# hgyhungry/ge-spmm

Measured on AMD Instinct MI355X. Metric: SpMM GFLOP/s (= 2*nnz*N/t), CSR x dense fp32, N=128, higher is better.
Workload: dtype f32

## Files before the change

### gespmm_amd/csrc/plan.cpp

```cpp

#include <hip/hip_runtime.h>

#include <algorithm>
#include <atomic>
#include <chrono>
#include <cstdio>
#include <cstdlib>
#include <cstring>
#include <memory>
#include <new>
#include <vector>

#include "../../include/gespmm.h"
#include "auto_plan.h"
#include "plan.h"
#include "plan_device.h"
#include "plan_policy.h"
#include "reorder.h"
#include "sddmm_heads.h"
#include "select.h"
#include "spmm_device.h"
#include "spmm_heads.h"
#include "spmm_kernels.h"

// ... 141 lines not shown
void drop_plan_copy(gespmm_plan* p) {
    if (p->d_block) (void)hipFree(p->d_block);
    if (p->d_tasks) (void)hipFree(p->d_tasks);
    p->d_block = nullptr;
    p->d_perm = p->d_rowptr = p->d_colind = p->d_src_begin = p->d_tasks = p->d_gtasks = nullptr;
    p->d_val = nullptr;
    p->ntasks = p->ngtasks = 0;
}

hipError_t permute_values(const gespmm_plan* p, const float* val, hipStream_t st) {
    hipLaunchKernelGGL(permute_values_kernel, dim3((unsigned)((p->nnz + 255) / 256)), dim3(256), 0, st, p->d_rowptr, p->d_src_begin, val,
                       p->d_val, (int)p->M, (int)p->nnz);
    return hipGetLastError();
}

gespmm::ClusterOptions cluster_options_from_env() {
    gespmm::ClusterOptions o;
    if (const char* v = getenv("GESPMM_CLUSTER_LEVELS")) o.max_levels = atoi(v);
    if (const char* v = getenv("GESPMM_CLUSTER_SWEEPS")) o.sweeps = atoi(v);
    if (const char* v = getenv("GESPMM_CLUSTER_STOP")) o.stop_percent = atoi(v);
    if (const char* v = getenv("GESPMM_CLUSTER_CAP")) o.first_cap = atoi(v);
    return o;
}

gespmm::ClusterOptions cluster_options_for(const gespmm::PlanFacts& f, int threads) {
    gespmm::ClusterOptions o = cluster_options_from_env();
    if (o.max_levels <= 0) o.max_levels = gespmm::cluster_levels_for(f);
    if (o.sweeps <= 0) o.sweeps = gespmm::cluster_sweeps_for(f);
    o.threads = threads;
    return o;
}

void lap(hipStream_t st, const char* what) {
    static const bool timing = getenv("GESPMM_PLAN_TIMING") != nullptr;
    if (!timing) return;
    (void)hipStreamSynchronize(st);
    static thread_local std::chrono::steady_clock::time_point last;
    const auto now = std::chrono::steady_clock::now();
    if (what) fprintf(stderr, "[plan] %-22s %8.3f ms\n", what, std::chrono::duration<double>(now - last).count() * 1e3);
    last = now;
}

gespmm::RouteAnswer route_of(const gespmm_plan* p, int64_t N, int reduce, bool operands_aligned16) {
// ... 42 lines not shown
}

namespace gespmm {
bool plan_is_clustered(const gespmm_plan* p) { return p && p->reordered; }
static std::atomic<bool> g_analysis_warm{false};
bool analysis_is_warm() { return g_analysis_warm.load(std::memory_order_relaxed); }
void mark_analysis_warm() { g_analysis_warm.store(true, std::memory_order_relaxed); }
}

extern "C" {

int gespmm_cluster_rows(const int32_t* rowptr, const int32_t* colind, int64_t M, int64_t K, int32_t threads,
                        int32_t* perm_out, int32_t* levels_out, int32_t* clusters_out ) {
    if (M < 0 || K < 0 || (M > 0 && (!rowptr || !perm_out))) return GESPMM_EINVAL;
    gespmm::ClusterOptions opt;
    opt.threads = threads;
    gespmm::ClusterStats st;
    try {
        if (gespmm::cluster_rows(M, K, rowptr, colind, opt, perm_out, &st) != 0) return GESPMM_EINVAL;
    } catch (const std::bad_alloc&) {
        return GESPMM_ENOMEM;
    }
    if (levels_out) *levels_out = st.levels;
    if (clusters_out)
        for (int i = 0; i < 16; ++i) clusters_out[i] = st.clusters[i];
    return 0;
}

int gespmm_cluster_rows_study(const int32_t* rowptr, const int32_t* colind, int64_t M, int64_t K, int32_t max_levels, int32_t sweeps,
                              int32_t* perm_out, int32_t* top_label_out, int32_t* clusters_out ) {
// ... 19 lines not shown
}

int gespmm_device_cluster_rows(const int32_t* rowptr, const int32_t* colind, int64_t M, int64_t K, int64_t nnz,
                               int32_t* perm_out_host, int32_t* levels_out, int32_t* clusters_out , void* stream) {
    if (M < 0 || K < 0 || nnz < 0 || (M > 0 && (!rowptr || !perm_out_host)) || (nnz > 0 && !colind)) return GESPMM_EINVAL;
    if (M == 0) return 0;
    hipStream_t st = reinterpret_cast<hipStream_t>(stream);
    int32_t max_deg = 0, bad = 0;
    hipError_t e = gespmm::device_validate_csr(rowptr, colind, M, K, nnz, &max_deg, &bad, nullptr, st);
    if (e != hipSuccess) return (int)e;
    if (bad) return GESPMM_EINVAL;
    int32_t* d_perm = nullptr;
    e = hipMalloc(reinterpret_cast<void**>(&d_perm), (size_t)M * 4);
    if (e != hipSuccess) return (int)e;
    gespmm::ClusterOptions opt;
    gespmm::ClusterStats stats;
    e = gespmm::device_cluster_rows(M, K, nnz, rowptr, colind, opt, d_perm, &stats, st);
    if (e == hipSuccess) e = hipMemcpyAsync(perm_out_host, d_perm, (size_t)M * 4, hipMemcpyDeviceToHost, st);
    if (e == hipSuccess) e = hipStreamSynchronize(st);
    (void)hipFree(d_perm);
    if (e != hipSuccess) return (int)e;
    if (levels_out) *levels_out = stats.levels;
    if (clusters_out)
        for (int i = 0; i < 16; ++i) clusters_out[i] = stats.clusters[i];
    return 0;
}

double gespmm_device_l2_model(const int32_t* rowptr, const int32_t* colind, int64_t M, int64_t K, int64_t nnz,
                              const int32_t* perm_host, int32_t slices, int64_t window_rows, int64_t max_entries_per_slice,
                              int32_t samples_per_slice, void* stream) {
// ... 1001 lines not shown
    if (p->heads_last_route >= 0) {
        const size_t used = strlen(kern);
        char geo[64] = "";
        if (p->heads_last_route != 0)
            snprintf(geo, sizeof geo, " V=%d S=%d W=%d", p->heads_last_geo.vec, p->heads_last_geo.strips, p->heads_last_geo.group);
        snprintf(kern + used, sizeof kern - used, " | heads H=%lld F=%lld route=%d (%s%s)", (long long)p->heads_last_H, (long long)p->heads_last_F,
                 p->heads_last_route, p->heads_last_route == 1 ? (p->reordered ? "heads kernel, task table" : "heads kernel") : "per-head composition",
                 geo);
    }
    int n;
    if (p->reordered) {
        char lv[128] = "";
        int off = 0;
        for (int i = 0; i < p->stats.levels && i < 16 && off < 100; ++i)
            off += snprintf(lv + off, sizeof lv - (size_t)off, "%s%d", i ? ">" : "", p->stats.clusters[i]);
        char tuned[200] = "";
        if (p->tuned)
            snprintf(tuned, sizeof tuned, " tuned[us: batch-stream=%.1f segmented-stream=%.1f staged-rows=%.1f batch-stream-V4=%.1f padded-records=%.1f]",
                     p->tune_us[0], p->tune_us[1], p->tune_us[2], p->tune_us[3], p->tune_us[4]);
        n = snprintf(out, (size_t)capacity,
                     "order=%s levels=%d clusters=%s tasks=%d task_entries=%d group_tasks=%d max_degree=%d probe=%.3f l2_model=%.3f->%.3f "
                     "analysis=%.4fs on the %s (clustering %.4fs)%s | %s",
                     p->identity_order ? "storage(plan copy: as local as the clustering)" : "clustered", p->stats.levels, lv, p->ntasks, p->task_entries,
                     p->ngtasks, p->max_degree, p->facts.wedge_probe, p->hits_before,
                     p->hits_after, p->analysis_seconds, p->analysis == GESPMM_PLAN_ANALYSIS_HOST ? "host" : "device", p->cluster_seconds, tuned, kern);
    } else {
        char why[200] = "";
        if (p->cost_skipped)
            snprintf(why, sizeof why, " (analysis skipped: est. gain %.1f us x %d launches < est. cost %.0f us; wedge probe %.4f)", p->est_gain_us,
                     p->facts.expected_launches > 0 ? p->facts.expected_launches : gespmm::kDefaultExpectedLaunches, p->est_cost_us,
                     p->facts.wedge_probe);
        n = snprintf(out, (size_t)capacity, "order=storage max_degree=%d l2_model=%.3f->%.3f analysis=%.4fs%s | %s",
                     p->max_degree, p->hits_before, p->hits_after, p->analysis_seconds, why, kern);
    }
    return gespmm::describe_result(n, capacity);
}

void gespmm_release_cached_memory(void) { gespmm::release_cached_arena(); }
// ... 13 lines not shown
```

### gespmm_amd/csrc/plan_device.hip

```cpp

#include <hip/hip_runtime.h>
#include <stdint.h>

#include <algorithm>
#include <chrono>
#include <atomic>
#include <mutex>
#include <cstdio>
#include <cstdlib>
#include <vector>

#include <rocprim/device/device_radix_sort.hpp>
#include <rocprim/block/block_scan.hpp>
#include <rocprim/device/device_scan.hpp>
#include <rocprim/device/device_segmented_radix_sort.hpp>
#include <rocprim/functional.hpp>

#include "auto_plan.h"
#include "plan_device.h"
#include "spmm_device.h"
#include "spmm_kernels.h"
#include "workspace.h"

namespace gespmm {
// ... 347 lines not shown
    if (threadIdx.x < kBins) s_base[threadIdx.x] = s_cnt[threadIdx.x] > 0 ? atomicAdd(&counts[threadIdx.x], s_cnt[threadIdx.x]) : 0;
    __syncthreads();
    if (b >= 0) lists[(int64_t)b * n + s_base[b] + off] = i;
}

struct LpArgs {
    DAdj adj;
    const int32_t* nbr_label;
    const int32_t* cur;
    int32_t* next;
    const int32_t* size;
    const int32_t* rweight;
    long long cap;
    uint32_t seed;
    int skip_half;
    const int32_t* list;
    const int32_t* count;
    const int32_t* done;
};

__device__ inline bool sits_out(const LpArgs& a, int node) {
    return a.skip_half && (mix32((uint32_t)node * 0x85ebca6bu ^ a.seed) & 1u);
}

template <int G>
__device__ inline void best_of_group(long long& bt, uint32_t& bh, int& bL) {
#pragma unroll
    for (int o = G / 2; o > 0; o >>= 1) {
        const long long ot = __shfl_xor(bt, o, G);
        const uint32_t oh = (uint32_t)__shfl_xor((int)bh, o, G);
        const int oL = __shfl_xor(bL, o, G);
        if (ot > bt || (ot == bt && ot >= 0 && oh < bh)) {
            bt = ot;
            bh = oh;
// ... 15 lines not shown
        L = a.nbr_label[a.adj.idx[e]];
        wt = (L >= 0) ? (a.adj.w ? a.adj.w[e] : 1) : 0;
    }
    long long tot = 0;
#pragma unroll
    for (int j = 0; j < G; ++j) {
        const int Lj = __shfl(L, j, G);
        const int wj = __shfl(wt, j, G);
        tot += (Lj == L) ? wj : 0;
    }
    const int own = active ? a.cur[node] : -1;
    long long own_w = (L >= 0 && L == own) ? tot : 0;
#pragma unroll
    for (int o = G / 2; o > 0; o >>= 1) own_w = max(own_w, __shfl_xor(own_w, o, G));
    bool cand = L >= 0 && L != own && tot > own_w;
    if (ROWS && cand) cand = (long long)a.size[L] + a.rweight[node] <= a.cap;
    long long bt = cand ? tot : -1;
    uint32_t bh = mix32((uint32_t)L ^ a.seed);
    int bL = L;
    best_of_group<G>(bt, bh, bL);
    if (active && l == 0) a.next[node] = (ROWS && sits_out(a, node)) ? own : (bt >= 0 ? bL : own);
}

struct LpSmallClasses {
    const int32_t* lists;
    const int32_t* counts;
    int n_side;
    int blk_end[4];
};
template <bool ROWS>
// ... 48 lines not shown
        int slot = (int)(mix32((uint32_t)own) & (uint32_t)(T - 1));
        for (;;) {
            const int k = s_key[slot];
            if (k == own) {
                own_w = (long long)s_wt[slot];
                break;
            }
            if (k == -1) break;
            slot = (slot + 1) & (T - 1);
        }
    }
    long long bt = -1;
    uint32_t bh = 0;
    int bL = -1;
    const int rw = ROWS ? a.rweight[node] : 0;
    for (int s = lane; s < T; s += 64) {
        const int L = s_key[s];
        if (L < 0 || L == own) continue;
        const long long t = (long long)s_wt[s];
        if (t <= own_w) continue;
        if (ROWS && (long long)a.size[L] + rw > a.cap) continue;
        const uint32_t h = mix32((uint32_t)L ^ a.seed);
        if (t > bt || (t == bt && h < bh)) {
            bt = t;
            bh = h;
            bL = L;
        }
    }
    best_of_group<64>(bt, bh, bL);
    if (lane == 0) a.next[node] = bt >= 0 ? bL : own;
}

template <bool ROWS>
__global__ void __launch_bounds__(256) k_lp_dense(LpArgs a, unsigned long long* __restrict__ acc_all, int64_t nlabels) {
    __shared__ long long s_t[256];
// ... 11 lines not shown
            continue;
        }
        const int beg = a.adj.ptr[node], end = a.adj.ptr[node + 1];
        for (int e = beg + tid; e < end; e += 256) {
            const int L = a.nbr_label[a.adj.idx[e]];
            if (L >= 0) atomicAdd(&acc[L], (unsigned long long)(a.adj.w ? a.adj.w[e] : 1));
        }
        __threadfence();
        __syncthreads();
        const long long own_w =
            own >= 0 ? (long long)__hip_atomic_load(&acc[own], __ATOMIC_RELAXED, __HIP_MEMORY_SCOPE_AGENT) : 0;
        long long bt = -1;
        uint32_t bh = 0;
        int bL = -1;
        const int rw = ROWS ? a.rweight[node] : 0;
        for (int e = beg + tid; e < end; e += 256) {
            const int L = a.nbr_label[a.adj.idx[e]];
            if (L < 0 || L == own) continue;
            const long long t = (long long)__hip_atomic_load(&acc[L], __ATOMIC_RELAXED, __HIP_MEMORY_SCOPE_AGENT);
            if (t <= own_w) continue;
            if (ROWS && (long long)a.size[L] + rw > a.cap) continue;
            const uint32_t h = mix32((uint32_t)L ^ a.seed);
            if (t > bt || (t == bt && h < bh)) {
                bt = t;
                bh = h;
                bL = L;
            }
        }
        s_t[tid] = bt;
        s_h[tid] = bh;
        s_L[tid] = bL;
        __syncthreads();
        for (int o = 128; o > 0; o >>= 1) {
            if (tid < o) {
                const long long ot = s_t[tid + o];
// ... 12 lines not shown
            if (L >= 0) __hip_atomic_store(&acc[L], 0ull, __ATOMIC_RELAXED, __HIP_MEMORY_SCOPE_AGENT);
        }
        __threadfence();
        __syncthreads();
    }
}

__global__ void k_commit_cols(int32_t* __restrict__ cur, const int32_t* __restrict__ next, const int32_t* __restrict__ twin,
                              const int32_t* __restrict__ rlab, int n, const int32_t* __restrict__ done) {
    if (*done) return;
    const int i = blockIdx.x * blockDim.x + threadIdx.x;
    if (i < n) cur[i] = (twin && twin[i] >= 0) ? rlab[twin[i]] : next[i];
}

__global__ void k_commit_rows(int32_t* __restrict__ cur, const int32_t* __restrict__ next, const int32_t* __restrict__ rweight,
                              int32_t* __restrict__ size, int n, int32_t* __restrict__ changed, int32_t* __restrict__ ticket,
                              int32_t* __restrict__ done) {
    if (*done) return;
    const int i = blockIdx.x * blockDim.x + threadIdx.x;
    int ch = 0;
    if (i < n) {
        const int v = next[i], old = cur[i];
        if (v != old) {
            ch = 1;
            cur[i] = v;
            const int w = rweight[i];
            atomicAdd(&size[v], w);
            atomicSub(&size[old], w);
        }
    }
    __shared__ int s_changed;
    if (threadIdx.x == 0) s_changed = 0;
    __syncthreads();
    const unsigned long long m = __ballot(ch);
    if (m && lane_id() == (__ffsll((long long)m) - 1)) atomicAdd(&s_changed, __popcll(m));
    __syncthreads();
    if (threadIdx.x == 0) {
        if (s_changed) atomicAdd(changed, s_changed);
        __threadfence();
        if (atomicAdd(ticket, 1) == (int)gridDim.x - 1) {
            const int c = atomicAdd(changed, 0);
            if ((long long)c * 400 < n) atomicExch(done, 1);
            atomicExch(changed, 0);
            atomicExch(ticket, 0);
        }
    }
}


__global__ void k_mark_used(const int32_t* __restrict__ rlab, int R, const int32_t* __restrict__ clab, int C,
                            int32_t* __restrict__ used_r, int32_t* __restrict__ used_c) {
    const int i = blockIdx.x * blockDim.x + threadIdx.x;
    if (i < R) used_r[rlab[i]] = 1;
    if (i < C) {
        const int L = clab[i];
        if (L >= 0) used_c[L] = 1;
// ... 11 lines not shown

__global__ void k_level_init(int32_t* __restrict__ rlab, int32_t* __restrict__ rnext, int32_t* __restrict__ size,
                             const int32_t* __restrict__ rweight, int R, int32_t* __restrict__ clab,
                             int32_t* __restrict__ cnext, int C, int32_t* __restrict__ flags ) {
    const int i = blockIdx.x * blockDim.x + threadIdx.x;
    if (i < R) {
        rlab[i] = i;
        rnext[i] = i;
        size[i] = rweight[i];
    }
    if (i < C) {
        clab[i] = -1;
        cnext[i] = -1;
    }
    if (i < 16) flags[i] = 0;
}

__global__ void k_fill2(int32_t* __restrict__ a, int64_t na, int32_t va, int32_t* __restrict__ b, int64_t nb, int32_t vb) {
    const int64_t i = (int64_t)blockIdx.x * blockDim.x + threadIdx.x;
    if (i < na) a[i] = va;
    if (i < nb) b[i] = vb;
}

__global__ void k_parents(const int32_t* __restrict__ rlab, const int32_t* __restrict__ rid, int R,
                          int32_t* __restrict__ parent) {
    const int r = blockIdx.x * blockDim.x + threadIdx.x;
    if (r < R) parent[r] = rid[rlab[r]];
}

__global__ void k_new_weights(const int32_t* __restrict__ rlab, const int32_t* __restrict__ rid,
// ... 507 lines not shown
    lv.region = Scratch::kLevelA;
    GESPMM_TRY(build_cols(sc, lv, nullptr, st));
    {
        int32_t* rw = nullptr;
        sc.use(lv.region);
        GESPMM_TRY(sc.get(&rw, M));
        hipLaunchKernelGGL(k_fill, dim3(grid_for(M)), dim3(256), 0, st, rw, M, 1);
        lv.rweight = rw;
    }
    std::vector<int32_t*> parents;
    std::vector<int32_t> parent_count;
    std::vector<int32_t> cluster_count;

    int32_t* flags_dev = nullptr;
    static_assert(4 + 2 * kBins <= 16, "k_level_init zeroes 16 flags");
    sc.use(Scratch::kPersist);
    GESPMM_TRY(sc.get(&flags_dev, 16));

    long long cap = opt.first_cap > 0 ? opt.first_cap : 256;
    const int max_levels = opt.max_levels > 0 ? opt.max_levels : kDefaultClusterLevels;
    const int sweeps = opt.sweeps > 0 ? opt.sweeps : 5;
    const int stop_percent = opt.stop_percent > 0 ? opt.stop_percent : 97;

    static const bool timing = getenv("GESPMM_PLAN_TIMING") != nullptr;
    auto lap = [&](const char* what, int level) {
        if (!timing) return;
        (void)hipStreamSynchronize(st);
        static thread_local std::chrono::steady_clock::time_point last;
        const auto now = std::chrono::steady_clock::now();
        if (what) fprintf(stderr, "[plan]   L%d %-16s %8.3f ms\n", level, what, std::chrono::duration<double>(now - last).count() * 1e3);
        last = now;
    };
    lap(nullptr, 0);
    for (int level = 0; level < max_levels; ++level) {
        const int32_t R = lv.R, C = lv.C;
        if (R <= 1 || lv.E == 0) break;
        lap("(cols/setup)", level);
        sc.reset(Scratch::kTemp);
        sc.use(Scratch::kTemp);
        int32_t *rlab = nullptr, *clab = nullptr, *rnext = nullptr, *cnext = nullptr, *size = nullptr, *rlists = nullptr,
                *clists = nullptr;
        GESPMM_TRY(sc.get(&rlab, R));
        GESPMM_TRY(sc.get(&clab, C));
        const size_t after_labels = sc.mark();
        GESPMM_TRY(sc.get(&rnext, R));
        GESPMM_TRY(sc.get(&cnext, C));
        GESPMM_TRY(sc.get(&size, R));
        GESPMM_TRY(sc.get(&rlists, (int64_t)kBins * R));
        GESPMM_TRY(sc.get(&clists, (int64_t)kBins * C));
        hipLaunchKernelGGL(k_level_init, dim3(grid_for(std::max(R, C))), dim3(256), 0, st, rlab, rnext, size, lv.rweight, R, clab,
                           cnext, C, flags_dev);
        int32_t* done = flags_dev;
        int32_t* changed = flags_dev + 1;
        int32_t* ticket = flags_dev + 2;
        int32_t* rcounts = flags_dev + 4;
        int32_t* ccounts = flags_dev + 4 + kBins;
        hipLaunchKernelGGL(k_bin_nodes, dim3((unsigned)((R + kBinThreads - 1) / kBinThreads)), dim3(kBinThreads), 0, st, lv.rows.ptr,
                           (const int32_t*)nullptr, R, rlists, rcounts);
        hipLaunchKernelGGL(k_bin_nodes, dim3((unsigned)((C + kBinThreads - 1) / kBinThreads)), dim3(kBinThreads), 0, st, lv.cols.ptr,
                           lv.twin, C, clists, ccounts);
        GESPMM_TRY(hipGetLastError());
        int32_t h_counts[2 * kBins];
        GESPMM_TRY(fetch(h_counts, (const int32_t*)(flags_dev + 4), 2 * kBins, st));
        unsigned long long* acc = nullptr;
        int acc_wgs = 0;
        if (h_counts[kBins - 1] > 0 || h_counts[2 * kBins - 1] > 0) {
            const int want = std::max(h_counts[kBins - 1], h_counts[2 * kBins - 1]);
            int64_t wgs = std::min<int64_t>(want, 64);
            while (wgs > 1 && wgs * (int64_t)R * 8 > (1ll << 30)) wgs >>= 1;
            acc_wgs = (int)wgs;
            GESPMM_TRY(sc.get(&acc, (int64_t)acc_wgs * R));
            GESPMM_TRY(hipMemsetAsync(acc, 0, (size_t)acc_wgs * (size_t)R * 8, st));
        }
        const bool twins = lv.twin != nullptr;
        for (int sweep = 0; sweep < sweeps; ++sweep) {
            LpArgs a;
            a.seed = 0x9e3779b9u * (uint32_t)(level * 16 + sweep + 1);
            a.done = done;
            a.cap = cap;
            a.list = nullptr;
            a.count = nullptr;
            a.adj = lv.cols;
            a.nbr_label = rlab;
            a.cur = clab;
            a.next = cnext;
            a.size = nullptr;
            a.rweight = nullptr;
            a.skip_half = 0;
            GESPMM_TRY(launch_half_sweep<false>(a, clists, ccounts, h_counts + kBins, C, acc, acc_wgs, R, st));
            hipLaunchKernelGGL(k_commit_cols, dim3(grid_for(C)), dim3(256), 0, st, clab, (const int32_t*)cnext, lv.twin,
                               (const int32_t*)rlab, C, (const int32_t*)done);
            a.adj = lv.rows;
            a.nbr_label = clab;
            a.cur = rlab;
            a.next = rnext;
            a.size = size;
            a.rweight = lv.rweight;
            a.skip_half = (twins && sweep + 1 < sweeps) ? 1 : 0;
            GESPMM_TRY(launch_half_sweep<true>(a, rlists, rcounts, h_counts, R, acc, acc_wgs, R, st));
            hipLaunchKernelGGL(k_commit_rows, dim3((unsigned)((R + 1023) / 1024)), dim3(1024), 0, st, rlab, (const int32_t*)rnext,
                               lv.rweight, size, R, changed, ticket, done);
            GESPMM_TRY(hipGetLastError());
        }
        lap("sweeps", level);
        sc.rewind(Scratch::kTemp, after_labels);

        int32_t *used = nullptr, *pos = nullptr, *rid = nullptr, *cid = nullptr, *parent = nullptr;
        const int64_t R1 = (int64_t)R + 1;
        sc.use(Scratch::kPersist);
        GESPMM_TRY(sc.get(&parent, R));
        sc.use(Scratch::kTemp);
        GESPMM_TRY(sc.get(&rid, R));
        GESPMM_TRY(sc.get(&cid, R));
        const size_t after_ids = sc.mark();
        GESPMM_TRY(sc.get(&used, 2 * R1));
        GESPMM_TRY(sc.get(&pos, 2 * R1));
        GESPMM_TRY(hipMemsetAsync(used, 0, (size_t)(2 * R1) * 4, st));
        hipLaunchKernelGGL(k_mark_used, dim3(grid_for(std::max(R, C))), dim3(256), 0, st, (const int32_t*)rlab, R,
                           (const int32_t*)clab, C, used, used + R1);
        GESPMM_TRY(exclusive_scan<int32_t>(sc, used, pos, 2 * R1, st));
        hipLaunchKernelGGL(k_make_ids, dim3(grid_for(R)), dim3(256), 0, st, (const int32_t*)used, (const int32_t*)pos,
                           (const int32_t*)(pos + R), R, rid, cid);
        hipLaunchKernelGGL(k_parents, dim3(grid_for(R)), dim3(256), 0, st, (const int32_t*)rlab, (const int32_t*)rid, R, parent);
        GESPMM_TRY(hipGetLastError());
        int32_t tot[2] = {0, 0};
        GESPMM_TRY(hipMemcpyAsync(&tot[0], pos + R, 4, hipMemcpyDeviceToHost, st));
        GESPMM_TRY(hipMemcpyAsync(&tot[1], pos + 2 * R1 - 1, 4, hipMemcpyDeviceToHost, st));
        GESPMM_TRY(hipStreamSynchronize(st));
        const int32_t R2 = tot[0], C2 = tot[1] - tot[0];
        sc.rewind(Scratch::kTemp, after_ids);
        parents.push_back(parent);
        parent_count.push_back(R);
        cluster_count.push_back(R2);
        if (stats) {
            stats->levels = level + 1;
            if (level < 16) stats->clusters[level] = R2;
        }
        lap("relabel", level);
        const bool last = (R2 <= 8 || (int64_t)R2 * 100 > (int64_t)R * stop_percent || level + 1 >= max_levels);
        if (last) break;

        DLevel nx;
        nx.R = R2;
        nx.C = C2;
        nx.region = lv.region == Scratch::kLevelA ? Scratch::kLevelB : Scratch::kLevelA;
        sc.reset(nx.region);
        int32_t *rw2 = nullptr, *twin2 = nullptr;
        sc.use(nx.region);
        GESPMM_TRY(sc.get(&rw2, R2));
        GESPMM_TRY(sc.get(&twin2, C2));
        sc.use(Scratch::kTemp);
// ... 806 lines not shown
```

### gespmm_amd/csrc/plan_policy.cpp

```cpp

#include <cstdlib>
#include "plan_policy.h"

#include <cstddef>
#include <cstring>

#include "../../include/gespmm.h"
#include "select.h"
#include "spmm_kernels.h"

namespace gespmm {

int long_row_flags(int64_t M, int64_t nnz, int32_t max_degree, int user_flags) {
    const int64_t mean = M > 0 ? (nnz + M - 1) / M : 0;
    int64_t threshold = 32 * mean;
    if (threshold < kLongRowThreshold) threshold = kLongRowThreshold;
    const bool plain_would = nnz >= kLongRowMinNnz || (nnz >= (1 << 20) && M > 0 && nnz / M >= 8);
    if (!(user_flags & (GESPMM_FLAG_STRICT_ORDER | GESPMM_FLAG_SPLIT_LONG_ROWS)))
        user_flags |= (plain_would && max_degree > threshold) ? GESPMM_FLAG_SPLIT_LONG_ROWS : GESPMM_FLAG_STRICT_ORDER;
    return user_flags;
}

static bool crc_family(int v) { return v >= GESPMM_VARIANT_CRC && v <= GESPMM_VARIANT_CRC_CWM8; }
static bool deep_analysis(const PlanFacts& f);
// ... 1 lines not shown
CostEstimate estimate_analysis_cost(const PlanFacts& f) {
    CostEstimate c;
    if (f.wedge_probe < 0.0) c.hits_gain = 0.60;
    else {
        double r = 0.0, x = f.wedge_probe;
        if (x > 0.0) {
            r = x < 1.0 ? 1.0 : x;
            for (int i = 0; i < 40; ++i) r = 0.5 * (r + x / r);
        }
        c.hits_gain = 0.10 + 0.90 * r;
        if (c.hits_gain > 0.85) c.hits_gain = 0.85;
    }
    const double gathered_mb = 4.0 * (double)f.nnz * (double)f.N / 1e6;
    c.gain_us = gathered_mb * c.hits_gain * 0.085;
    const double e = (double)f.nnz;
    c.cost_us = !deep_analysis(f) ? 3300.0 + 0.55e-3 * e : 5000.0 + 0.6e-3 * e;
    if (f.host_analysis) c.cost_us *= 30.0;
    if (f.cold_start && !f.host_analysis) c.cost_us += 29000.0;
    return c;
}

bool analysis_could_pay(int64_t M, int64_t K, int64_t nnz, int64_t N, int expected_launches) {
    if (M <= 0 || nnz <= 0 || N <= 0) return false;
    PlanFacts f;
    f.M = M;
    f.K = K;
    f.nnz = nnz;
    f.N = N;
    f.expected_launches = expected_launches;
    f.wedge_probe = 1.0;
    f.cold_start = false;
// ... 34 lines not shown
    const int64_t rowb = 4 * (f.N < f.tile_cols ? f.N : f.tile_cols);
    a.model_window = (3ll << 20) / (rowb > 0 ? rowb : 4);
    return a;
}

static bool deep_analysis(const PlanFacts& f) {
    const long long launches = f.expected_launches > 0 ? f.expected_launches : kDefaultExpectedLaunches;
    return launches * (long long)(f.N > 0 ? f.N : 1) >= 100000ll;
}

int cluster_levels_for(const PlanFacts& f) { return deep_analysis(f) ? 0 : 3; }

int cluster_sweeps_for(const PlanFacts& f) {
    const long long launches = f.expected_launches > 0 ? f.expected_launches : kDefaultExpectedLaunches;
    return launches * (long long)(f.N > 0 ? f.N : 1) >= 12800ll ? 0 : 3;
}

int model_points_for(const PlanFacts& f) {
    return deep_analysis(f) ? 4096 : 1024;
}

bool keep_clustered_order(const PlanFacts& f, const AnalysisDecision& a, double hits_before, double hits_after) {
    if (f.reorder_mode != GESPMM_PLAN_REORDER_AUTO) return true;
    if (hits_after < hits_before + 0.03) return false;
    if (a.dense_try && hits_after < 0.65) return false;
    return true;
}

static int default_task_entries(int64_t N) {
    const int64_t row_bytes = 4 * (N < 256 ? N : 256);
// ... 316 lines not shown
```

### gespmm_amd/csrc/plan_policy.h

```cpp
#pragma once
#include <stdint.h>

#include "../../include/gespmm.h"
#include "spmm_kernels.h"

namespace gespmm {

struct PlanFacts {
    int64_t M = 0, K = 0, nnz = 0, N = 0;
    int variant = -1;
    int sel_variant = 0;
    bool slab_blocked = false;
    int64_t tile_cols = 0;
    int32_t max_degree = 0;
    int reorder_mode = 0;
    int kernel_choice = 0;
    bool host_analysis = false;
    int user_flags = 0;
    int opt_task_entries = 0, opt_row_floor = 0;
    int expected_launches = 0;
    bool cold_start = false;
    double wedge_probe = -1.0;

    int64_t mean_ceil() const { return M > 0 ? (nnz + M - 1) / M : 0; }
// ... 15 lines not shown

struct AnalysisDecision {
    int launch_flags = 0;
    bool cost_skipped = false;
    CostEstimate cost;
    bool analyse = false;
    bool dense_try = false;
    int64_t model_window = 0;
    int64_t model_sample = 0;
};
AnalysisDecision decide_analysis(const PlanFacts& f);
bool analysis_could_pay(int64_t M, int64_t K, int64_t nnz, int64_t N, int expected_launches);

int cluster_levels_for(const PlanFacts& f);
int cluster_sweeps_for(const PlanFacts& f);
int model_points_for(const PlanFacts& f);
int staged_rows_for(const PlanFacts& f, const StagedShape& shape);
int staged_fill_window(const PlanFacts& f, const StagedShape& shape);

bool keep_clustered_order(const PlanFacts& f, const AnalysisDecision& a, double hits_before, double hits_after);

struct PlanKernelDecision {
    int task_entries = 0;
    int group_task_entries = 0;
    int64_t row_floor = 0;
    bool build_staged = false;
    bool shallow_unroll = false;
};
PlanKernelDecision choose_plan_kernel(const PlanFacts& f, double hits_after);

// ... 45 lines not shown
```

### gespmm_amd/csrc/reorder.cpp

```cpp

#include "reorder.h"

#include <algorithm>
#include <cstdint>
#include <cstring>
#include <numeric>
#include <thread>
#if defined(__linux__)
#include <pthread.h>
#include <sched.h>
#endif
#include <vector>

namespace gespmm {

namespace {

inline uint32_t mix32(uint32_t x) {
    x ^= x >> 16;
    x *= 0x7feb352du;
    x ^= x >> 15;
    x *= 0x846ca68bu;
    x ^= x >> 16;
    return x;
// ... 81 lines not shown
    int32_t best = own;
    int64_t best_w = (own >= 0) ? acc[own] : 0;
    uint32_t best_h = 0;
    bool best_is_own = true;
    for (int32_t L : touched) {
        if (L == own) continue;
        const int64_t w = acc[L];
        if (w < best_w || (best_is_own && w == best_w)) continue;
        if (!allowed(L)) continue;
        const uint32_t h = mix32((uint32_t)L ^ seed);
        if (w > best_w || h < best_h) {
            best = L;
            best_w = w;
            best_h = h;
            best_is_own = false;
        }
    }
    for (int32_t L : touched) acc[L] = 0;
    return best;
}

}

int cluster_rows(int64_t M, int64_t K, const int32_t* rowptr, const int32_t* colind, const ClusterOptions& opt,
                 int32_t* perm, ClusterStats* stats, int32_t* top_labels) {
    if (M < 0 || K < 0 || (M > 0 && (!rowptr || !perm))) return -1;
    if (stats) *stats = ClusterStats{};
    if (M == 0) return 0;
    const int64_t nnz = rowptr[M];
    if (nnz < 0 || (nnz > 0 && !colind)) return -1;
// ... 32 lines not shown
                }
                lv.rows.ptr[r + 1] = (int64_t)lv.rows.idx.size();
            }
        }
    }
    transpose(lv.rows, lv.R, lv.C, lv.cols);
    lv.rweight.assign((size_t)M, 1);

    std::vector<int32_t> node_of_row((size_t)M);
    std::iota(node_of_row.begin(), node_of_row.end(), 0);
    std::vector<std::vector<int32_t>> level_labels;

    int64_t cap = opt.first_cap > 0 ? opt.first_cap : 256;
    const int max_levels = opt.max_levels > 0 ? opt.max_levels : 6;
    const int sweeps = opt.sweeps > 0 ? opt.sweeps : 5;

    for (int level = 0; level < max_levels; ++level) {
        const int32_t R = lv.R, C = lv.C;
        if (R <= 1 || lv.rows.ptr[R] == 0) break;
        std::vector<int32_t> rlab((size_t)R), clab((size_t)C, -1), next((size_t)std::max(R, C));
        std::iota(rlab.begin(), rlab.end(), 0);
        std::vector<int64_t> size((size_t)R);
        std::vector<std::vector<int64_t>> acc((size_t)threads);
        std::vector<std::vector<int32_t>> touched((size_t)threads);
        for (int sweep = 0; sweep < sweeps; ++sweep) {
            const uint32_t seed = 0x9e3779b9u * (uint32_t)(level * 16 + sweep + 1);
            const bool twins = !lv.twin.empty();
            parallel_for(C, threads, [&](int64_t lo, int64_t hi, int t) {
                if (acc[t].empty()) acc[t].assign((size_t)R, 0);
                for (int64_t c = lo; c < hi; ++c) {
                    if (twins && lv.twin[c] >= 0) next[c] = rlab[lv.twin[c]];
                    else
                        next[c] = heaviest_label(lv.cols, c, rlab.data(), clab[c], seed, acc[t], touched[t],
                                                 [](int32_t) { return true; });
                }
            });
            std::copy(next.begin(), next.begin() + C, clab.begin());
            std::fill(size.begin(), size.end(), 0);
            for (int32_t r = 0; r < R; ++r) size[rlab[r]] += lv.rweight[r];
            std::vector<int64_t> changed_t((size_t)threads, 0);
            parallel_for(R, threads, [&](int64_t lo, int64_t hi, int t) {
                if (acc[t].empty()) acc[t].assign((size_t)R, 0);
                int64_t ch = 0;
                for (int64_t r = lo; r < hi; ++r) {
                    const int64_t w = lv.rweight[r];
                    const int32_t own = rlab[r];
                    if (twins && sweep + 1 < sweeps && (mix32((uint32_t)r * 0x85ebca6bu ^ seed) & 1u)) {
                        next[r] = own;
                        continue;
                    }
                    const int32_t L = heaviest_label(lv.rows, r, clab.data(), own, seed, acc[t], touched[t],
                                                     [&](int32_t cand) { return size[cand] + w <= cap; });
                    next[r] = L;
                    ch += (L != own);
                }
                changed_t[t] = ch;
            });
            std::copy(next.begin(), next.begin() + R, rlab.begin());
            int64_t changed = 0;
            for (int64_t c : changed_t) changed += c;
            if (changed * 400 < R) break;
        }
        std::vector<int32_t> rid((size_t)R, -1), cid((size_t)R + 1, -1);
        int32_t R2 = 0, C2 = 0;
        for (int32_t r = 0; r < R; ++r) rid[rlab[r]] = 0;
        for (int32_t L = 0; L < R; ++L)
            if (rid[L] == 0) rid[L] = R2++;
        for (int32_t c = 0; c < C; ++c)
            if (clab[c] >= 0) cid[clab[c]] = 0;
        for (int32_t L = 0; L < R; ++L)
            if (cid[L] == 0) cid[L] = C2++;
        for (int64_t r = 0; r < M; ++r) node_of_row[r] = rid[rlab[node_of_row[r]]];
        level_labels.push_back(node_of_row);
        if (stats) {
            stats->levels = level + 1;
            if (level < 16) stats->clusters[level] = R2;
        }
        if (R2 <= 8 || (int64_t)R2 * 100 > (int64_t)R * (opt.stop_percent > 0 ? opt.stop_percent : 97)) break;
        Level nx;
        nx.R = R2;
        nx.C = C2;
        nx.rweight.assign((size_t)R2, 0);
        std::vector<int64_t> mptr((size_t)R2 + 1, 0);
        for (int32_t r = 0; r < R; ++r) {
            const int32_t n = rid[rlab[r]];
            mptr[(size_t)n + 1]++;
            nx.rweight[n] += lv.rweight[r];
        }
        for (int32_t n = 0; n < R2; ++n) mptr[n + 1] += mptr[n];
        std::vector<int32_t> members((size_t)R);
        {
// ... 123 lines not shown
```

### gespmm_amd/csrc/reorder.h

```cpp
#pragma once
#include <stdint.h>

namespace gespmm {

struct ClusterOptions {
    int threads = 0;
    int max_levels = 0;
    int sweeps = 0;
    int64_t first_cap = 0;
    int cap_growth = 0;
    int stop_percent = 0;
};

struct ClusterStats {
    int levels = 0;
    int32_t clusters[16] = {0};
};

int cluster_rows(int64_t M, int64_t K, const int32_t* rowptr, const int32_t* colind, const ClusterOptions& opt,
                 int32_t* perm, ClusterStats* stats, int32_t* top_labels = nullptr );

double simulate_l2_hits(int64_t M, int64_t K, const int32_t* rowptr, const int32_t* colind, const int32_t* perm,
                        int slices, int64_t window, int64_t max_entries_per_slice = 0);

}
```

Before: 5888.

## Add modularity-gain refinement to row clustering on coarse levels

```diff
diff --git a/gespmm_amd/csrc/plan.cpp b/gespmm_amd/csrc/plan.cpp
--- a/gespmm_amd/csrc/plan.cpp
+++ b/gespmm_amd/csrc/plan.cpp
@@ -179,8 +179,15 @@
     return hipGetLastError();
 }
 
+void refine_options_from_env(gespmm::ClusterOptions& o) {
+    if (const char* v = getenv("GESPMM_CLUSTER_REFINE")) o.refine = atoi(v) != 0 ? 1 : 0;
+    if (const char* v = getenv("GESPMM_CLUSTER_REFINE_SWEEPS")) o.refine_sweeps = atoi(v);
+    if (const char* v = getenv("GESPMM_CLUSTER_REFINE_BUDGET")) o.refine_budget = atoll(v);
+}
+
 gespmm::ClusterOptions cluster_options_from_env() {
     gespmm::ClusterOptions o;
+    refine_options_from_env(o);
     if (const char* v = getenv("GESPMM_CLUSTER_LEVELS")) o.max_levels = atoi(v);
     if (const char* v = getenv("GESPMM_CLUSTER_SWEEPS")) o.sweeps = atoi(v);
     if (const char* v = getenv("GESPMM_CLUSTER_STOP")) o.stop_percent = atoi(v);
@@ -192,6 +199,7 @@
     gespmm::ClusterOptions o = cluster_options_from_env();
     if (o.max_levels <= 0) o.max_levels = gespmm::cluster_levels_for(f);
     if (o.sweeps <= 0) o.sweeps = gespmm::cluster_sweeps_for(f);
+    if (o.refine < 0) o.refine = gespmm::cluster_refine_for(f);
     o.threads = threads;
     return o;
 }
@@ -264,6 +272,7 @@
                         int32_t* perm_out, int32_t* levels_out, int32_t* clusters_out ) {
     if (M < 0 || K < 0 || (M > 0 && (!rowptr || !perm_out))) return GESPMM_EINVAL;
     gespmm::ClusterOptions opt;
+    refine_options_from_env(opt);
     opt.threads = threads;
     gespmm::ClusterStats st;
     try {
@@ -313,6 +322,7 @@
     e = hipMalloc(reinterpret_cast<void**>(&d_perm), (size_t)M * 4);
     if (e != hipSuccess) return (int)e;
     gespmm::ClusterOptions opt;
+    refine_options_from_env(opt);
     gespmm::ClusterStats stats;
     e = gespmm::device_cluster_rows(M, K, nnz, rowptr, colind, opt, d_perm, &stats, st);
     if (e == hipSuccess) e = hipMemcpyAsync(perm_out_host, d_perm, (size_t)M * 4, hipMemcpyDeviceToHost, st);
@@ -1344,14 +1354,20 @@
         int off = 0;
         for (int i = 0; i < p->stats.levels && i < 16 && off < 100; ++i)
             off += snprintf(lv + off, sizeof lv - (size_t)off, "%s%d", i ? ">" : "", p->stats.clusters[i]);
+        char refine[160] = "refine=off";
+        if (p->stats.refined > 0) {
+            int ro = snprintf(refine, sizeof refine, "refine=modularity(%d levels) sweeps=", p->stats.refined);
+            for (int i = 0; i < p->stats.levels && i < 16 && ro < 140; ++i)
+                ro += snprintf(refine + ro, sizeof refine - (size_t)ro, "%s%d", i ? ">" : "", p->stats.sweeps[i]);
+        }
         char tuned[200] = "";
         if (p->tuned)
             snprintf(tuned, sizeof tuned, " tuned[us: batch-stream=%.1f segmented-stream=%.1f staged-rows=%.1f batch-stream-V4=%.1f padded-records=%.1f]",
                      p->tune_us[0], p->tune_us[1], p->tune_us[2], p->tune_us[3], p->tune_us[4]);
         n = snprintf(out, (size_t)capacity,
-                     "order=%s levels=%d clusters=%s tasks=%d task_entries=%d group_tasks=%d max_degree=%d probe=%.3f l2_model=%.3f->%.3f "
+                     "order=%s levels=%d clusters=%s %s tasks=%d task_entries=%d group_tasks=%d max_degree=%d probe=%.3f l2_model=%.3f->%.3f "
                      "analysis=%.4fs on the %s (clustering %.4fs)%s | %s",
-                     p->identity_order ? "storage(plan copy: as local as the clustering)" : "clustered", p->stats.levels, lv, p->ntasks, p->task_entries,
+                     p->identity_order ? "storage(plan copy: as local as the clustering)" : "clustered", p->stats.levels, lv, refine, p->ntasks, p->task_entries,
                      p->ngtasks, p->max_degree, p->facts.wedge_probe, p->hits_before,
                      p->hits_after, p->analysis_seconds, p->analysis == GESPMM_PLAN_ANALYSIS_HOST ? "host" : "device", p->cluster_seconds, tuned, kern);
     } else {
diff --git a/gespmm_amd/csrc/plan_device.hip b/gespmm_amd/csrc/plan_device.hip
--- a/gespmm_amd/csrc/plan_device.hip
+++ b/gespmm_amd/csrc/plan_device.hip
@@ -385,10 +385,17 @@
     long long cap;
     uint32_t seed;
     int skip_half;
+    const int32_t* kdeg;
+    const int32_t* vol;
+    const long long* W;
     const int32_t* list;
     const int32_t* count;
     const int32_t* done;
 };
+
+__device__ inline long long move_gain(const LpArgs& a, long long t, long long own_w, long long k, long long own_vol, int L, long long W) {
+    return (t - own_w) * W - k * ((long long)a.vol[L] - own_vol);
+}
 
 __device__ inline bool sits_out(const LpArgs& a, int node) {
     return a.skip_half && (mix32((uint32_t)node * 0x85ebca6bu ^ a.seed) & 1u);
@@ -434,6 +441,14 @@
 #pragma unroll
     for (int o = G / 2; o > 0; o >>= 1) own_w = max(own_w, __shfl_xor(own_w, o, G));
     bool cand = L >= 0 && L != own && tot > own_w;
+    if (ROWS && a.vol) {
+        cand = L >= 0 && L != own;
+        if (cand) {
+            const long long k = a.kdeg[node];
+            tot = move_gain(a, tot, own_w, k, (long long)a.vol[own] - k, L, *a.W);
+            cand = tot > 0;
+        }
+    }
     if (ROWS && cand) cand = (long long)a.size[L] + a.rweight[node] <= a.cap;
     long long bt = cand ? tot : -1;
     uint32_t bh = mix32((uint32_t)L ^ a.seed);
@@ -512,11 +527,16 @@
     uint32_t bh = 0;
     int bL = -1;
     const int rw = ROWS ? a.rweight[node] : 0;
+    const bool gains = ROWS && a.vol;
+    const long long k = gains ? a.kdeg[node] : 0, own_vol = gains ? (long long)a.vol[own] - k : 0, W = gains ? *a.W : 0;
     for (int s = lane; s < T; s += 64) {
         const int L = s_key[s];
         if (L < 0 || L == own) continue;
-        const long long t = (long long)s_wt[s];
-        if (t <= own_w) continue;
+        long long t = (long long)s_wt[s];
+        if (gains) {
+            t = move_gain(a, t, own_w, k, own_vol, L, W);
+            if (t <= 0) continue;
+        } else if (t <= own_w) continue;
         if (ROWS && (long long)a.size[L] + rw > a.cap) continue;
         const uint32_t h = mix32((uint32_t)L ^ a.seed);
         if (t > bt || (t == bt && h < bh)) {
@@ -558,11 +578,16 @@
         uint32_t bh = 0;
         int bL = -1;
         const int rw = ROWS ? a.rweight[node] : 0;
+        const bool gains = ROWS && a.vol;
+        const long long k = gains ? a.kdeg[node] : 0, own_vol = gains ? (long long)a.vol[own] - k : 0, W = gains ? *a.W : 0;
         for (int e = beg + tid; e < end; e += 256) {
             const int L = a.nbr_label[a.adj.idx[e]];
             if (L < 0 || L == own) continue;
-            const long long t = (long long)__hip_atomic_load(&acc[L], __ATOMIC_RELAXED, __HIP_MEMORY_SCOPE_AGENT);
-            if (t <= own_w) continue;
+            long long t = (long long)__hip_atomic_load(&acc[L], __ATOMIC_RELAXED, __HIP_MEMORY_SCOPE_AGENT);
+            if (gains) {
+                t = move_gain(a, t, own_w, k, own_vol, L, W);
+                if (t <= 0) continue;
+            } else if (t <= own_w) continue;
             if (ROWS && (long long)a.size[L] + rw > a.cap) continue;
             const uint32_t h = mix32((uint32_t)L ^ a.seed);
             if (t > bt || (t == bt && h < bh)) {
@@ -605,8 +630,9 @@
 }
 
 __global__ void k_commit_rows(int32_t* __restrict__ cur, const int32_t* __restrict__ next, const int32_t* __restrict__ rweight,
-                              int32_t* __restrict__ size, int n, int32_t* __restrict__ changed, int32_t* __restrict__ ticket,
-                              int32_t* __restrict__ done) {
+                              int32_t* __restrict__ size, const int32_t* __restrict__ kdeg, int32_t* __restrict__ vol, int n,
+                              int32_t* __restrict__ changed, int32_t* __restrict__ ticket, int32_t* __restrict__ done,
+                              int32_t* __restrict__ sweeps_run) {
     if (*done) return;
     const int i = blockIdx.x * blockDim.x + threadIdx.x;
     int ch = 0;
@@ -618,6 +644,11 @@
             const int w = rweight[i];
             atomicAdd(&size[v], w);
             atomicSub(&size[old], w);
+            if (vol) {
+                const int k = kdeg[i];
+                atomicAdd(&vol[v], k);
+                atomicSub(&vol[old], k);
+            }
         }
     }
     __shared__ int s_changed;
@@ -631,6 +662,7 @@
         __threadfence();
         if (atomicAdd(ticket, 1) == (int)gridDim.x - 1) {
             const int c = atomicAdd(changed, 0);
+            atomicAdd(sweeps_run, 1);
             if ((long long)c * 400 < n) atomicExch(done, 1);
             atomicExch(changed, 0);
             atomicExch(ticket, 0);
@@ -672,6 +704,25 @@
         cnext[i] = -1;
     }
     if (i < 16) flags[i] = 0;
+}
+
+__global__ void __launch_bounds__(256) k_row_degrees(DAdj rows, int R, int32_t* __restrict__ kdeg, int32_t* __restrict__ vol,
+                                                     unsigned long long* __restrict__ W) {
+    __shared__ unsigned long long s_sum;
+    if (threadIdx.x == 0) s_sum = 0ull;
+    __syncthreads();
+    const int r = blockIdx.x * blockDim.x + threadIdx.x;
+    long long k = 0;
+    if (r < R) {
+        for (int e = rows.ptr[r]; e < rows.ptr[r + 1]; ++e) k += rows.w[e];
+        kdeg[r] = (int32_t)k;
+        vol[r] = (int32_t)k;
+    }
+#pragma unroll
+    for (int o = 32; o > 0; o >>= 1) k += __shfl_xor(k, o);
+    if (lane_id() == 0 && k) atomicAdd(&s_sum, (unsigned long long)k);
+    __syncthreads();
+    if (threadIdx.x == 0 && s_sum) atomicAdd(W, s_sum);
 }
 
 __global__ void k_fill2(int32_t* __restrict__ a, int64_t na, int32_t va, int32_t* __restrict__ b, int64_t nb, int32_t vb) {
@@ -1209,13 +1260,18 @@
 
     int32_t* flags_dev = nullptr;
     static_assert(4 + 2 * kBins <= 16, "k_level_init zeroes 16 flags");
+    unsigned long long* total_weight = nullptr;
     sc.use(Scratch::kPersist);
     GESPMM_TRY(sc.get(&flags_dev, 16));
+    GESPMM_TRY(sc.get(&total_weight, 1));
 
     long long cap = opt.first_cap > 0 ? opt.first_cap : 256;
     const int max_levels = opt.max_levels > 0 ? opt.max_levels : kDefaultClusterLevels;
     const int sweeps = opt.sweeps > 0 ? opt.sweeps : 5;
     const int stop_percent = opt.stop_percent > 0 ? opt.stop_percent : 97;
+    bool refine_on = cluster_refine_on(opt);
+    const int refine_sweeps = opt.refine_sweeps > 0 ? opt.refine_sweeps : 16;
+    const long long refine_budget = opt.refine_budget > 0 ? opt.refine_budget : 6144;
 
     static const bool timing = getenv("GESPMM_PLAN_TIMING") != nullptr;
     auto lap = [&](const char* what, int level) {
@@ -1234,7 +1290,8 @@
         sc.reset(Scratch::kTemp);
         sc.use(Scratch::kTemp);
         int32_t *rlab = nullptr, *clab = nullptr, *rnext = nullptr, *cnext = nullptr, *size = nullptr, *rlists = nullptr,
-                *clists = nullptr;
+                *clists = nullptr, *kdeg = nullptr, *vol = nullptr;
+        bool refine = refine_on && lv.twin != nullptr;
         GESPMM_TRY(sc.get(&rlab, R));
         GESPMM_TRY(sc.get(&clab, C));
         const size_t after_labels = sc.mark();
@@ -1243,6 +1300,12 @@
         GESPMM_TRY(sc.get(&size, R));
         GESPMM_TRY(sc.get(&rlists, (int64_t)kBins * R));
         GESPMM_TRY(sc.get(&clists, (int64_t)kBins * C));
+        if (refine) {
+            GESPMM_TRY(sc.get(&kdeg, R));
+            GESPMM_TRY(sc.get(&vol, R));
+            GESPMM_TRY(hipMemsetAsync(total_weight, 0, 8, st));
+            hipLaunchKernelGGL(k_row_degrees, dim3(grid_for(R)), dim3(256), 0, st, lv.rows, R, kdeg, vol, total_weight);
+        }
         hipLaunchKernelGGL(k_level_init, dim3(grid_for(std::max(R, C))), dim3(256), 0, st, rlab, rnext, size, lv.rweight, R, clab,
                            cnext, C, flags_dev);
         int32_t* done = flags_dev;
@@ -1256,7 +1319,15 @@
                            lv.twin, C, clists, ccounts);
         GESPMM_TRY(hipGetLastError());
         int32_t h_counts[2 * kBins];
+        unsigned long long h_weight = 0;
+        if (refine && level == 1) GESPMM_TRY(hipMemcpyAsync(&h_weight, total_weight, 8, hipMemcpyDeviceToHost, st));
         GESPMM_TRY(fetch(h_counts, (const int32_t*)(flags_dev + 4), 2 * kBins, st));
+        if (refine && level == 1 && (long long)h_weight * 2 > (long long)nnz) {
+            refine = refine_on = false;
+            kdeg = vol = nullptr;
+        }
+        const int level_sweeps = refine ? refine_sweeps : sweeps;
+        const long long level_cap = refine ? std::max<long long>(refine_budget, opt.first_cap) : cap;
         unsigned long long* acc = nullptr;
         int acc_wgs = 0;
         if (h_counts[kBins - 1] > 0 || h_counts[2 * kBins - 1] > 0) {
@@ -1268,11 +1339,14 @@
             GESPMM_TRY(hipMemsetAsync(acc, 0, (size_t)acc_wgs * (size_t)R * 8, st));
         }
         const bool twins = lv.twin != nullptr;
-        for (int sweep = 0; sweep < sweeps; ++sweep) {
+        for (int sweep = 0; sweep < level_sweeps; ++sweep) {
             LpArgs a;
-            a.seed = 0x9e3779b9u * (uint32_t)(level * 16 + sweep + 1);
+            a.seed = 0x9e3779b9u * (uint32_t)(refine ? level * 64 + sweep + 257 : level * 16 + sweep + 1);
             a.done = done;
-            a.cap = cap;
+            a.cap = level_cap;
+            a.kdeg = nullptr;
+            a.vol = nullptr;
+            a.W = nullptr;
             a.list = nullptr;
             a.count = nullptr;
             a.adj = lv.cols;
@@ -1291,10 +1365,13 @@
             a.next = rnext;
             a.size = size;
             a.rweight = lv.rweight;
-            a.skip_half = (twins && sweep + 1 < sweeps) ? 1 : 0;
+            a.skip_half = (twins && (refine || sweep + 1 < sweeps)) ? 1 : 0;
+            a.kdeg = kdeg;
+            a.vol = vol;
+            a.W = reinterpret_cast<const long long*>(total_weight);
             GESPMM_TRY(launch_half_sweep<true>(a, rlists, rcounts, h_counts, R, acc, acc_wgs, R, st));
             hipLaunchKernelGGL(k_commit_rows, dim3((unsigned)((R + 1023) / 1024)), dim3(1024), 0, st, rlab, (const int32_t*)rnext,
-                               lv.rweight, size, R, changed, ticket, done);
+                               lv.rweight, size, (const int32_t*)kdeg, vol, R, changed, ticket, done, flags_dev + 3);
             GESPMM_TRY(hipGetLastError());
         }
         lap("sweeps", level);
@@ -1319,6 +1396,8 @@
         hipLaunchKernelGGL(k_parents, dim3(grid_for(R)), dim3(256), 0, st, (const int32_t*)rlab, (const int32_t*)rid, R, parent);
         GESPMM_TRY(hipGetLastError());
         int32_t tot[2] = {0, 0};
+        int32_t sweeps_run = 0;
+        GESPMM_TRY(hipMemcpyAsync(&sweeps_run, flags_dev + 3, 4, hipMemcpyDeviceToHost, st));
         GESPMM_TRY(hipMemcpyAsync(&tot[0], pos + R, 4, hipMemcpyDeviceToHost, st));
         GESPMM_TRY(hipMemcpyAsync(&tot[1], pos + 2 * R1 - 1, 4, hipMemcpyDeviceToHost, st));
         GESPMM_TRY(hipStreamSynchronize(st));
@@ -1329,7 +1408,11 @@
         cluster_count.push_back(R2);
         if (stats) {
             stats->levels = level + 1;
-            if (level < 16) stats->clusters[level] = R2;
+            if (level < 16) {
+                stats->clusters[level] = R2;
+                stats->sweeps[level] = sweeps_run;
+            }
+            stats->refined += refine ? 1 : 0;
         }
         lap("relabel", level);
         const bool last = (R2 <= 8 || (int64_t)R2 * 100 > (int64_t)R * stop_percent || level + 1 >= max_levels);
diff --git a/gespmm_amd/csrc/plan_policy.cpp b/gespmm_amd/csrc/plan_policy.cpp
--- a/gespmm_amd/csrc/plan_policy.cpp
+++ b/gespmm_amd/csrc/plan_policy.cpp
@@ -39,7 +39,7 @@
     const double gathered_mb = 4.0 * (double)f.nnz * (double)f.N / 1e6;
     c.gain_us = gathered_mb * c.hits_gain * 0.085;
     const double e = (double)f.nnz;
-    c.cost_us = !deep_analysis(f) ? 3300.0 + 0.55e-3 * e : 5000.0 + 0.6e-3 * e;
+    c.cost_us = !deep_analysis(f) ? 3300.0 + 0.55e-3 * e : 5000.0 + 1.1e-3 * e;
     if (f.host_analysis) c.cost_us *= 30.0;
     if (f.cold_start && !f.host_analysis) c.cost_us += 29000.0;
     return c;
@@ -104,6 +104,10 @@
 int cluster_sweeps_for(const PlanFacts& f) {
     const long long launches = f.expected_launches > 0 ? f.expected_launches : kDefaultExpectedLaunches;
     return launches * (long long)(f.N > 0 ? f.N : 1) >= 12800ll ? 0 : 3;
+}
+
+int cluster_refine_for(const PlanFacts& f) {
+    return deep_analysis(f) ? 1 : 0;
 }
 
 int model_points_for(const PlanFacts& f) {
diff --git a/gespmm_amd/csrc/plan_policy.h b/gespmm_amd/csrc/plan_policy.h
--- a/gespmm_amd/csrc/plan_policy.h
+++ b/gespmm_amd/csrc/plan_policy.h
@@ -53,6 +53,7 @@
 
 int cluster_levels_for(const PlanFacts& f);
 int cluster_sweeps_for(const PlanFacts& f);
+int cluster_refine_for(const PlanFacts& f);
 int model_points_for(const PlanFacts& f);
 int staged_rows_for(const PlanFacts& f, const StagedShape& shape);
 int staged_fill_window(const PlanFacts& f, const StagedShape& shape);
diff --git a/gespmm_amd/csrc/reorder.cpp b/gespmm_amd/csrc/reorder.cpp
--- a/gespmm_amd/csrc/reorder.cpp
+++ b/gespmm_amd/csrc/reorder.cpp
@@ -119,6 +119,37 @@
             best_w = w;
             best_h = h;
             best_is_own = false;
+        }
+    }
+    for (int32_t L : touched) acc[L] = 0;
+    return best;
+}
+
+template <typename Allowed>
+inline int32_t best_gain_label(const Adj& a, int64_t node, const int32_t* nbr_label, int32_t own, uint32_t seed, int64_t W,
+                               int64_t k, const int64_t* vol, std::vector<int64_t>& acc, std::vector<int32_t>& touched,
+                               Allowed&& allowed) {
+    touched.clear();
+    for (int64_t e = a.ptr[node]; e < a.ptr[node + 1]; ++e) {
+        const int32_t L = nbr_label[a.idx[e]];
+        if (L < 0) continue;
+        if (acc[L] == 0) touched.push_back(L);
+        acc[L] += a.w[e];
+    }
+    const int64_t own_w = acc[own], own_vol = vol[own] - k;
+    int32_t best = own;
+    int64_t best_g = 0;
+    uint32_t best_h = 0;
+    for (int32_t L : touched) {
+        if (L == own) continue;
+        const int64_t g = (acc[L] - own_w) * W - k * (vol[L] - own_vol);
+        if (g <= 0 || g < best_g) continue;
+        if (!allowed(L)) continue;
+        const uint32_t h = mix32((uint32_t)L ^ seed);
+        if (g > best_g || h < best_h) {
+            best = L;
+            best_g = g;
+            best_h = h;
         }
     }
     for (int32_t L : touched) acc[L] = 0;
@@ -181,17 +212,41 @@
     int64_t cap = opt.first_cap > 0 ? opt.first_cap : 256;
     const int max_levels = opt.max_levels > 0 ? opt.max_levels : 6;
     const int sweeps = opt.sweeps > 0 ? opt.sweeps : 5;
+    bool refine_on = cluster_refine_on(opt);
+    const int64_t entries0 = (int64_t)lv.rows.idx.size();
+    const int refine_sweeps = opt.refine_sweeps > 0 ? opt.refine_sweeps : 16;
+    const int64_t refine_budget = opt.refine_budget > 0 ? opt.refine_budget : 6144;
 
     for (int level = 0; level < max_levels; ++level) {
         const int32_t R = lv.R, C = lv.C;
         if (R <= 1 || lv.rows.ptr[R] == 0) break;
+        bool refine = refine_on && !lv.twin.empty();
+        std::vector<int64_t> kdeg, vol;
+        int64_t W = 0;
+        if (refine) {
+            kdeg.assign((size_t)R, 0);
+            vol.assign((size_t)R, 0);
+            parallel_for(R, threads, [&](int64_t lo, int64_t hi, int) {
+                for (int64_t r = lo; r < hi; ++r) {
+                    int64_t k = 0;
+                    for (int64_t e = lv.rows.ptr[r]; e < lv.rows.ptr[r + 1]; ++e) k += lv.rows.w[e];
+                    kdeg[r] = k;
+                }
+            });
+            for (int32_t r = 0; r < R; ++r) W += kdeg[r];
+            if (level == 1 && W * 2 > entries0) refine = refine_on = false;
+        }
+        const int level_sweeps = refine ? refine_sweeps : sweeps;
+        const int64_t level_cap = refine ? std::max<int64_t>(refine_budget, opt.first_cap) : cap;
         std::vector<int32_t> rlab((size_t)R), clab((size_t)C, -1), next((size_t)std::max(R, C));
         std::iota(rlab.begin(), rlab.end(), 0);
         std::vector<int64_t> size((size_t)R);
         std::vector<std::vector<int64_t>> acc((size_t)threads);
         std::vector<std::vector<int32_t>> touched((size_t)threads);
-        for (int sweep = 0; sweep < sweeps; ++sweep) {
-            const uint32_t seed = 0x9e3779b9u * (uint32_t)(level * 16 + sweep + 1);
+        int sweeps_run = 0;
+        for (int sweep = 0; sweep < level_sweeps; ++sweep) {
+            ++sweeps_run;
+            const uint32_t seed = 0x9e3779b9u * (uint32_t)(refine ? level * 64 + sweep + 257 : level * 16 + sweep + 1);
             const bool twins = !lv.twin.empty();
             parallel_for(C, threads, [&](int64_t lo, int64_t hi, int t) {
                 if (acc[t].empty()) acc[t].assign((size_t)R, 0);
@@ -205,6 +260,10 @@
             std::copy(next.begin(), next.begin() + C, clab.begin());
             std::fill(size.begin(), size.end(), 0);
             for (int32_t r = 0; r < R; ++r) size[rlab[r]] += lv.rweight[r];
+            if (refine) {
+                std::fill(vol.begin(), vol.end(), 0);
+                for (int32_t r = 0; r < R; ++r) vol[rlab[r]] += kdeg[r];
+            }
             std::vector<int64_t> changed_t((size_t)threads, 0);
             parallel_for(R, threads, [&](int64_t lo, int64_t hi, int t) {
                 if (acc[t].empty()) acc[t].assign((size_t)R, 0);
@@ -212,12 +271,15 @@
                 for (int64_t r = lo; r < hi; ++r) {
                     const int64_t w = lv.rweight[r];
                     const int32_t own = rlab[r];
-                    if (twins && sweep + 1 < sweeps && (mix32((uint32_t)r * 0x85ebca6bu ^ seed) & 1u)) {
+                    if (twins && (refine || sweep + 1 < sweeps) && (mix32((uint32_t)r * 0x85ebca6bu ^ seed) & 1u)) {
                         next[r] = own;
                         continue;
                     }
-                    const int32_t L = heaviest_label(lv.rows, r, clab.data(), own, seed, acc[t], touched[t],
-                                                     [&](int32_t cand) { return size[cand] + w <= cap; });
+                    const int32_t L =
+                        refine ? best_gain_label(lv.rows, r, clab.data(), own, seed, W, kdeg[r], vol.data(), acc[t], touched[t],
+                                                 [&](int32_t cand) { return size[cand] + w <= level_cap; })
+                               : heaviest_label(lv.rows, r, clab.data(), own, seed, acc[t], touched[t],
+                                                [&](int32_t cand) { return size[cand] + w <= cap; });
                     next[r] = L;
                     ch += (L != own);
                 }
@@ -241,7 +303,11 @@
         level_labels.push_back(node_of_row);
         if (stats) {
             stats->levels = level + 1;
-            if (level < 16) stats->clusters[level] = R2;
+            if (level < 16) {
+                stats->clusters[level] = R2;
+                stats->sweeps[level] = sweeps_run;
+            }
+            stats->refined += refine ? 1 : 0;
         }
         if (R2 <= 8 || (int64_t)R2 * 100 > (int64_t)R * (opt.stop_percent > 0 ? opt.stop_percent : 97)) break;
         Level nx;
diff --git a/gespmm_amd/csrc/reorder.h b/gespmm_amd/csrc/reorder.h
--- a/gespmm_amd/csrc/reorder.h
+++ b/gespmm_amd/csrc/reorder.h
@@ -10,11 +10,19 @@
     int64_t first_cap = 0;
     int cap_growth = 0;
     int stop_percent = 0;
+    int refine = -1;
+    int refine_sweeps = 0;
+    int64_t refine_budget = 0;
 };
+
+constexpr int kClusterRefineDefault = 1;
+inline bool cluster_refine_on(const ClusterOptions& o) { return (o.refine < 0 ? kClusterRefineDefault : o.refine) != 0; }
 
 struct ClusterStats {
     int levels = 0;
     int32_t clusters[16] = {0};
+    int32_t sweeps[16] = {0};
+    int refined = 0;
 };
 
 int cluster_rows(int64_t M, int64_t K, const int32_t* rowptr, const int32_t* colind, const ClusterOptions& opt,
```

Result: no change. 5882, median of 2 (-0.1%).
